# fmfi-compbio/nadavca

Measured on AMD Instinct MI355X. Metric: reads/sec (align_signal, ~4k-sample reads), higher is better.
Workload: dtype f64

## Files before the change

nadavca_amd/csrc/kernels_align3.hip:

```cpp
#include <math.h>

#include <new>
#include <vector>

#include "nvk_internal.h"
#include "xmath.h"
#include "dens.h"
#include "lane3.h"
#include "wave.h"

namespace {

using dens::density;
using dens::density_begin;
using dens::density_end;
using dens::DensHalf;
using dens::ETN;

constexpr int CH = 64;
static_assert(CH == 64, "a refill is one sample per lane");
constexpr int PF = 8;
constexpr int RU = 16;
constexpr int FT = 16;
static_assert(FT % PF == 0 && 32 % FT == 0, "forward trip");
// ... 805 lines not shown
    case 3: return !pair && set_sweeps<MEL, 3, false, TW>(k);
    case 4: return pair ? set_sweeps<MEL, 4, true, TW>(k) : set_sweeps<MEL, 4, false, TW>(k);
    case 5: return pair ? set_sweeps<MEL, 5, true, TW>(k) : set_sweeps<MEL, 5, false, TW>(k);
    default: return false;
  }
}

bool select_sweeps(int mel, bool pair, int W, int rsh, Align3Kernel k[2]) {
  switch (mel) {
    case 0: return sweeps_of<0>(pair, W, rsh, k);
    case 1: return sweeps_of<1>(pair, W, rsh, k);
    case 2: return sweeps_of<2>(pair, W, rsh, k);
    case 3: return sweeps_of<3>(pair, W, rsh, k);
    case 4: return sweeps_of<4>(pair, W, rsh, k);
    default: return false;
  }
}

}

int launch_align3(nvk_ctx *ctx, const BatchArgs &a, int transitions, const ReadMeta *metas, const PlanTotals &tot,
                  const int *order, const int32_t *steps_sorted, int32_t *out_events, int32_t *out_status,
                  int *d_retry) {
  static_assert(WS_OFFS < (int)(sizeof(ctx->ws) / sizeof(ctx->ws[0])), "workspace table too small");
  if (a.n_reads == 0) return NVK_OK;
  const int mel = a.mel;
  if (mel < 0 || mel > 4) {
    nvk_set_error("min_event_length %d outside the compiled range 0..4", mel);
    return NVK_ERR_UNSUPPORTED;
  }
  const int max_c = tot.max_c < 1 ? 1 : tot.max_c;
  int rc = nvk_ws_reserve(ctx, WS_MISC, 256);
  if (rc) return rc;
  int *counter = (int *)ctx->ws[WS_MISC];
  NVK_HIP(hipMemsetAsync(counter, 0, 2 * sizeof(int), ctx->stream));
  NVK_HIP(hipMemsetAsync(d_retry, 0, sizeof(int), ctx->stream));

  constexpr int C_HARD = 24;
  static_assert(ALIGN1_C_CAP + 4 < 8 && C_HARD + 4 < 32, "no kernel for the rescale period these skews need");
  struct Cls { int hi; int W; };
  Cls cls[2];
  int ncls = 0;
  const int64_t n_wide = (int64_t)tot.n_wide;
  const int max_cw = tot.max_cw < 1 ? 1 : tot.max_cw;
  if (a.n_reads - n_wide > 0 || max_c <= ALIGN1_C_CAP)
    cls[ncls++] = Cls{max_c < ALIGN1_C_CAP ? max_c : ALIGN1_C_CAP, 1};
  if (max_c > ALIGN1_C_CAP) cls[ncls++] = Cls{max_cw < C_HARD ? max_cw : C_HARD, ALIGN3_TEAM_W};
  rc = nvk_ws_reserve(ctx, WS_RSTATE, (size_t)a.n_reads * sizeof(int2));
  if (rc) return rc;
  TimerScope ts_align(ctx, NVK_K_ALIGN);
  for (int k = 0; k < ncls; k++) {
    int c = cls[k].hi;
    const int W = cls[k].W, TLk = 64 * W;
    auto lds_need = [&](int cc, int slot_bytes) {
      const int Hc = (cc + mel > 0 ? cc + mel : 1) + (W > 1 ? 1 : 0);
      int SRc = 256;
      while (SRc < 64 * cc + CH) SRc <<= 1;
      return (size_t)ETN * 8 + (size_t)W * SRc * 8 + (size_t)Hc * TLk * slot_bytes + slot_bytes + 16 + 12 * W;
    };
    while (c > 1 && lds_need(c, 20) > 160 * 1024) --c;
    int rsh = transitions ? 4 : 3;
    while ((1 << rsh) <= c + mel) rsh++;
    Align3Kernel kern[2];
    if (!select_sweeps(mel, transitions != 0, W, rsh, kern)) {
      nvk_set_error("no align3 kernel for min_event_length %d, transitions %d, %d waves, rescale period %d", mel,
                    transitions, W, 1 << rsh);
      return NVK_ERR_UNSUPPORTED;
    }
    const int H = (c + mel > 0 ? c + mel : 1) + (W > 1 ? 1 : 0);
    int SR = 256;
    while (SR < 64 * c + CH) SR <<= 1;
    const size_t lds = lds_need(c, 20);
    const size_t lds_rev = lds_need(c, 8);
    if (lds > 160 * 1024) return NVK_ERR_UNSUPPORTED;
    int per_cu = (int)((160 * 1024) / lds);
    if (per_cu > 4 * LB / W) per_cu = 4 * LB / W;
    if (per_cu < 1) per_cu = 1;
    int per_cu_rev = (int)((160 * 1024) / lds_rev);
    if (per_cu_rev > 4 * (W > 1 ? LB_REV_TEAM : LB_REV) / W) per_cu_rev = 4 * (W > 1 ? LB_REV_TEAM : LB_REV) / W;
    if (per_cu_rev < 1) per_cu_rev = 1;
    int32_t mxpad = 1;
    for (int64_t q = 0; q < a.n_reads; q++) mxpad = steps_sorted[q] > mxpad ? steps_sorted[q] : mxpad;
    const int64_t bp_stride = (int64_t)((mxpad + 31) / 32 + 1) * TLk;
    const int64_t cap = nvk_spill_cap(ctx, WS_SPILL);

    Align3Args g;
    g.metas = metas;
    g.fwdl = (const Lane3 *)ctx->ws[WS_LANE_F];
    g.revl = (const Lane3 *)ctx->ws[WS_LANE_R];
    g.offs = (const int32_t *)ctx->ws[WS_OFFS];
    g.signal = a.signal;
    g.bp_stride = bp_stride;
    g.counter = counter;
    g.order = order;
    g.H = H;
    g.SR = SR;
    g.transitions = transitions;
    g.c_cap = c;
    g.flag_above = (k == ncls - 1) ? 1 : 0;
    g.rstate = (int2 *)ctx->ws[WS_RSTATE];
    g.n_retry = d_retry;
    g.ties = (int32_t *)ctx->ws[WS_TIES];
    g.out_events = out_events;
    g.out_status = out_status;
    for (int ph = 0; ph < 2; ph++)
      if ((ph == 0 ? lds_rev : lds) > 64 * 1024)
        NVK_HIP(hipFuncSetAttribute((const void *)kern[ph], hipFuncAttributeMaxDynamicSharedMemorySize,
                                    (int)(ph == 0 ? lds_rev : lds)));
    const int64_t pos_lo = (W > 1) ? 0 : n_wide, pos_hi = (W > 1) ? n_wide : a.n_reads;
    int64_t lo = pos_lo;
    while (lo < pos_hi) {
      int64_t hi = lo, mx = 1;
      while (hi < pos_hi) {
        const int64_t m2 = steps_sorted[hi] > mx ? steps_sorted[hi] : mx;
        if (hi > lo && (m2 + 2 * PF) * 512 * W * (hi - lo + 1) > cap) break;
        mx = m2;
        ++hi;
      }
      int64_t n_chunk = hi - lo;
      int64_t spill_stride = (mx + 2 * PF) * 64;
      while ((rc = nvk_ws_reserve(ctx, WS_SPILL, (size_t)n_chunk * W * spill_stride * 8)) == NVK_ERR_NOMEM &&
             n_chunk > 1) {
        n_chunk = (n_chunk + 1) / 2;
        hi = lo + n_chunk;
        mx = 1;
        for (int64_t q = lo; q < hi; q++) mx = steps_sorted[q] > mx ? steps_sorted[q] : mx;
        spill_stride = (mx + 2 * PF) * 64;
      }
      if (rc) return rc;
      const int64_t L_stride = (mx >> rsh) + 4;
      rc = nvk_ws_reserve(ctx, WS_STAGE, (size_t)n_chunk * L_stride * 4);
      if (rc) return rc;
      int64_t slots_f = ctx->slots_override > 0 ? ctx->slots_override : (int64_t)ctx->num_cus * per_cu;
      int64_t slots_r = ctx->slots_override > 0 ? ctx->slots_override : (int64_t)ctx->num_cus * per_cu_rev;
      if (slots_f > n_chunk) slots_f = n_chunk;
      if (slots_r > n_chunk) slots_r = n_chunk;
      rc = nvk_ws_reserve(ctx, WS_BP, (size_t)slots_f * bp_stride * 4);
      if (rc) return rc;
      g.spill_v = (double *)ctx->ws[WS_SPILL];
      g.spill_L = (int32_t *)ctx->ws[WS_STAGE];
      g.bp = (uint32_t *)ctx->ws[WS_BP];
      g.spill_stride = spill_stride;
      g.L_stride = L_stride;
      g.n_reads = (int)n_chunk;
      g.read_lo = (int)lo;
      NVK_HIP(hipMemsetAsync(counter, 0, sizeof(int), ctx->stream));
      hipLaunchKernelGGL(kern[0], dim3((unsigned)slots_r), dim3(TLk), lds_rev, ctx->stream, g);
      NVK_HIP(hipMemsetAsync(counter, 0, sizeof(int), ctx->stream));
      hipLaunchKernelGGL(kern[1], dim3((unsigned)slots_f), dim3(TLk), lds, ctx->stream, g);
      NVK_HIP(hipGetLastError());
      lo = hi;
    }
  }
  ctx->last_spill_bytes = (int64_t)tot.steps * 64 * 16 + (int64_t)tot.steps / 16 * 8 + (int64_t)tot.steps * 8 * 2;
  return NVK_OK;
}
```

nadavca_amd/csrc/kernels_plan.hip:

```cpp
#include <math.h>

#include "nvk_internal.h"
#include "kmer.h"
#include "lane3.h"
#include "wave.h"

namespace {

__device__ __forceinline__ int read_is_bad(const DeviceModel &dm, const BatchArgs &a, int rd, int tid,
                                           int nthreads) {
  const int64_t s0 = a.sig_off[rd], s1 = a.sig_off[rd + 1], r0 = a.ref_off[rd], r1 = a.ref_off[rd + 1];
  const int64_t a0 = a.anc_off[rd], a1 = a.anc_off[rd + 1];
  const int64_t b0 = a.cb_off[rd], b1 = a.cb_off[rd + 1], c0 = a.ca_off[rd], c1 = a.ca_off[rd + 1];
  const int64_t N64 = s1 - s0, R64 = r1 - r0;
  if (s0 < 0 || r0 < 0 || a0 < 0 || b0 < 0 || c0 < 0 || a1 < a0 || b1 < b0 || c1 < c0 ||
      s1 > a.total_signal || r1 > a.total_ref || a1 > a.total_anchors || b1 - b0 > 0x3fffffff ||
      c1 - c0 > 0x3fffffff)
    return 1;
  if (R64 < 1 || N64 < 1 || N64 > 0x3fffffff || R64 > 0x1fffffff) return 1;
  const int R = (int)R64, A = (int)(a1 - a0), nb = (int)(b1 - b0), na = (int)(c1 - c0);
  const int32_t *anc = a.anchors + 2 * a0;
  const int32_t *ref = a.reference + r0, *cb = a.ctx_before + b0, *ca = a.ctx_after + c0;
  int bad = 0;
  for (int j = tid; j < A && !bad; j += nthreads) {
// ... 30 lines not shown
  }
  __syncthreads();
  int carry = 0;
  for (int base = 0; work && base <= R; base += 64) {
    int j = base + lane;
    int v = 0;
    if (j <= R) {
      unsigned long long w = tbs[j];
      v = (w >> 32) ? (int)(unsigned int)(w & 0xffffffffu) : 0;
    }
    v = max(wave_scan_max(v, lane), carry);
    carry = __shfl(v, 63, 64);
    if (j <= R) tbs[j] = (unsigned long long)(unsigned int)v;
  }
  carry = N;
  for (int base = (R / 64) * 64; work && base >= 0; base -= 64) {
    int j = base + lane;
    int v = N;
    if (j <= R) {
      unsigned long long w = tbe[j];
      v = (w >> 32) ? (int)(unsigned int)(w & 0xffffffffu) - 1 : N;
    } else {
      v = 0x7fffffff;
    }
    v = min(wave_scan_min_rev(v, lane), carry);
    carry = __shfl(v, 0, 64);
    if (j <= R) tbe[j] = (unsigned long long)(unsigned int)v;
  }
  __syncthreads();

}

constexpr int PLAN_T = 256;
__global__ __launch_bounds__(PLAN_T) void plan_kernel(DeviceModel dm, BatchArgs a, int mode,
                                                  double log_p_in, int c_cap, ReadMeta *metas,
                                                  RowParam *rows, unsigned long long *bandtmp,
                                                  PlanTotals *totals, Lane3 *lane_f, Lane3 *lane_r,
                                                  int32_t *lane_offs) {
  const int rd = blockIdx.x;
  const int tid = threadIdx.x, lane = tid & 63;
  __shared__ unsigned long long sh_cells;
  __shared__ int sh_c;
  if (rd >= a.n_reads) return;
  if (tid == 0) {
    sh_cells = 0ull;
    sh_c = 1;
  }
  const int64_t s0 = a.sig_off[rd], r0 = a.ref_off[rd], a0 = a.anc_off[rd];
  const int64_t N64 = a.sig_off[rd + 1] - s0;
  const int64_t R64 = a.ref_off[rd + 1] - r0;
  const int64_t A64 = a.anc_off[rd + 1] - a0;
  const int nb = (int)(a.cb_off[rd + 1] - a.cb_off[rd]);
  const int na = (int)(a.ca_off[rd + 1] - a.ca_off[rd]);
  const int32_t *ref = a.reference + r0;
  const int32_t *cb = a.ctx_before + a.cb_off[rd];
  const int32_t *ca = a.ctx_after + a.ca_off[rd];
  const int32_t *anc = a.anchors + 2 * a0;
  const int N = (int)N64, R = (int)R64, A = (int)A64;
  const int bw = a.bandwidth, mel = a.mel;

  ReadMeta m;
  m.sig_off = s0;
  m.ref_off = r0;
  m.N = N;
  m.R = R;
  m.status = NVK_READ_OK;
  m.pad = 0;
  m.cells = 0;
  m.cw = 0;
  m.rsv = 0;
  int T;
  if (mode == PLAN_ALIGN_TRANS) {
    T = 2 * R;
    m.row_off = 2 * r0;
  } else {
    T = R + 1;
    m.row_off = r0 + rd;
  }
  m.T = T;
  m.c = 1;
  m.t_min = 0;
  m.n_steps = 0;

  int bad = read_is_bad(dm, a, rd, tid, PLAN_T);
  bad = __syncthreads_or(bad);
  if (bad) {
    m.status = NVK_READ_BAD_INPUT;
    if (tid == 0) metas[rd] = m;
    return;
  }

  unsigned long long *tbs = bandtmp + 2 * (r0 + rd);
  unsigned long long *tbe = tbs + (R + 1);
  plan_bands(anc, A, R, N, bw, tbs, tbe, lane, tid < 64);

  RowParam *rp = rows + m.row_off;
  int badband = 0;
  int plateau = 0;
  long long cells = 0;
  for (int r = tid; r < T; r += PLAN_T) {
    RowParam p;
    int bidx = (mode == PLAN_ALIGN_TRANS) ? (r + 1) / 2 : r;
    p.bs = (int)(unsigned int)tbs[bidx];
    p.be = (int)(unsigned int)tbe[bidx];
    if (p.be < p.bs) badband = 1;
    cells += (long long)(p.be - p.bs + 1);
    p.lo = p.bs;
    p.hi = p.be;
    p.mean = 0.0;
    p.ac = 0.0;
    p.mc = 0.0;
    p.mel = 0;
    p.off = 0;
    if (r + 1 < T) {
      if (mode == PLAN_ALIGN_TRANS && (r & 1)) {
        int i = r / 2;
        double m1 = dm.mean[kmer_id(dm, ref, R, cb, nb, ca, na, i)];
        double m2 = dm.mean[kmer_id(dm, ref, R, cb, nb, ca, na, i + 1)];
        p.ac = (m1 == m2) ? -INFINITY : log_p_in;
        p.mel = 0;
        plateau |= (m1 == m2) ? 1 : 0;
      } else {
        int i = (mode == PLAN_ALIGN_TRANS) ? r / 2 : r;
        int64_t id = kmer_id(dm, ref, R, cb, nb, ca, na, i);
        p.mean = dm.mean[id];
        p.ac = dm.ac[id];
        p.mc = dm.mc[id];
        p.mel = mel;
      }
    }
    rp[r] = p;
  }
  badband = __syncthreads_or(badband);
  if (mode != PLAN_ALIGN_TRANS)
    for (int r = tid; r + 2 < T; r += PLAN_T) plateau |= (rp[r].mean == rp[r + 1].mean) ? 1 : 0;
  plateau = __syncthreads_or(plateau);
  cells = wave_sum(cells);
  if (lane == 0) atomicAdd(&sh_cells, (unsigned long long)cells);
  __syncthreads();

  int cneed = 1;
  for (int r = tid; r < T; r += PLAN_T) {
    int lo = rp[r].bs, hi = rp[r].be;
    if (r > 0) {
      int pm = rp[r - 1].mel;
      lo = min(lo, rp[r - 1].bs + pm) - max(pm - 1, 0);
    }
    if (r + 1 < T) {
      int pm = rp[r].mel;
      hi = max(hi, rp[r + 1].be - pm) + max(pm - 1, 0);
    }
    rp[r].lo = lo;
    rp[r].hi = hi;
  }
  __syncthreads();
  const int idle = (mode == PLAN_ALIGN_TRANS) ? 2 : 1;
  for (int r = 64 + tid; r < T; r += PLAN_T) {
    int d = rp[r - 64].hi - rp[r].lo + idle;
    if (d >= 0) cneed = max(cneed, d / 64 + 1);
  }
  cneed = max(cneed, max(mel - 1, 1));
  cneed = wave_max(cneed);
  if (lane == 0) atomicMax(&sh_c, cneed);
  __syncthreads();
  const int c = sh_c;
  cells = (long long)sh_cells;
  const bool team = (c > c_cap);
  int cw = 0;
  if (team) {
    constexpr int TL = 64 * ALIGN3_TEAM_W;
    __shared__ int sh_cw;
    if (tid == 0) sh_cw = max(mel - 1, 1);
    __syncthreads();
    int need = 1;
    for (int r = TL + tid; r < T; r += PLAN_T) {
      int d = rp[r - TL].hi - rp[r].lo + idle;
      if (d >= 0) need = max(need, d / TL + 1);
    }
    need = wave_max(need);
    if (lane == 0) atomicMax(&sh_cw, need);
    __syncthreads();
    cw = sh_cw;
  }

  constexpr int VT = 2048;
  __shared__ int sh_k[VT], sh_x[VT], sh_S[VT];
  __shared__ int sh_var;
  const int gmin = max(mel - 1, 1);
  const bool neg_gaps = (mode == PLAN_ALIGN_TRANS) && mel <= 2;
  if (tid == 0) sh_var = 0;
  __syncthreads();
  if (!team && T <= VT && T > 64 && (neg_gaps || c > gmin)) {
    for (int r = tid; r < T; r += PLAN_T) {
      int g = 0;
      if (r > 0) {
        g = gmin;
        if (neg_gaps) g = max(1 - rp[r - 1].mel, max(rp[r - 1].lo - rp[r].lo, rp[r - 1].hi - rp[r].hi));
        g = min(g, c);
      }
      sh_S[r] = g;
      sh_x[r] = 0;
    }
    __syncthreads();
    if (tid < 64) {
      int carry = 0;
      for (int b0 = 0; b0 < T; b0 += 64) {
        const int r = b0 + lane;
        const int v = wave_scan_add(r < T ? sh_S[r] : 0, lane) + carry;
        if (r < T) sh_S[r] = v;
        carry = __shfl(v, 63, 64);
      }
    }
    __syncthreads();
    for (int r = tid; r < T; r += PLAN_T)
      sh_k[r] = (r >= 64) ? rp[r - 64].hi - rp[r].lo + 1 + idle - (sh_S[r] - sh_S[r - 64]) : 0;
    __syncthreads();
    if (tid < 64) {
      const int NEG = -0x20000000;
      bool changed = true;
      int iter = 0;
      while (changed && iter < 64) {
        changed = false;
        ++iter;
        int carry = 0;
        for (int b0 = 0; b0 < T; b0 += 64) {
          const int r = b0 + lane;
          const int cur = r < T ? sh_x[r] : NEG;
          int v = cur;
          if (r < T && r >= 64) v = max(v, sh_x[r - 64] + sh_k[r]);
          v = max(wave_scan_max(v, lane), carry);
          if (r < T) {
            changed |= (v != cur);
            sh_x[r] = v;
          }
          carry = __shfl(v, 63, 64);
        }
        int carryz = NEG;
        for (int b0 = ((T - 1) / 64) * 64; b0 >= 0; b0 -= 64) {
          const int r = b0 + lane;
          const int cur = r < T ? sh_x[r] : 0;
          const int U = r < T ? c * r - sh_S[r] : 0;
          int z = r < T ? cur - U : NEG;
          z = max(-wave_scan_min_rev(-z, lane), carryz);
          if (r < T) {
            const int nx = z + U;
            changed |= (nx != cur);
            sh_x[r] = nx;
          }
          carryz = __shfl(z, 0, 64);
        }
        changed = __any(changed);
      }
      if (lane == 0) sh_var = changed ? 0 : 1;
    }
    __syncthreads();
  }
  const bool var_ok = (sh_var != 0);
  const int x0 = var_ok ? sh_x[0] : 0;
  const int cu = team ? cw : c;
  for (int r = tid; r < T; r += PLAN_T) rp[r].off = var_ok ? sh_x[r] - x0 + sh_S[r] : cu * r;
  const int off_top = var_ok ? sh_x[T - 1] - x0 + sh_S[T - 1] : cu * (T - 1);
  if (lane_f && !badband) {
    __syncthreads();
    lane3_rows(rp, T, N, cw, lane_f + m.row_off, lane_r + m.row_off, lane_offs + m.row_off, tid, PLAN_T);
  }

  if (tid == 0) {
    int t_min = rp[0].lo;
    int t_max = rp[T - 1].hi + c * (T - 1);
    m.c = c;
    m.cw = cw;
    m.t_min = t_min;
    m.n_steps = t_max - t_min + 1;
    m.pad = rp[T - 1].hi + off_top - t_min + 1;
    m.pad = (m.pad + 31) & ~31;
    m.cells = cells;
    m.rsv = plateau ? 1 : 0;
    if (badband) m.status = NVK_READ_BAD_BAND;
    metas[rd] = m;
    if (!badband) {
      atomicMax(&totals->max_steps, m.n_steps);
      atomicMax(&totals->max_c, c);
      atomicMax(&totals->max_cw, cw);
      if (c > c_cap) atomicAdd(&totals->n_wide, 1);
      atomicMax(&totals->max_T, T);
      atomicAdd(&totals->cells, (unsigned long long)cells);
      atomicAdd(&totals->steps, (unsigned long long)m.pad);
    }
  }
}


__global__ __launch_bounds__(64) void plan_ell_kernel(DeviceModel dm, BatchArgs a, int wobbling,
                                                      EllPlan pl, unsigned long long *bandtmp,
                                                      PlanTotals *totals) {
  const int rd = blockIdx.x;
  const int lane = threadIdx.x;
  if (rd >= a.n_reads) return;
  const int64_t s0 = a.sig_off[rd], r0 = a.ref_off[rd], a0 = a.anc_off[rd];
  const int64_t N64 = a.sig_off[rd + 1] - s0;
  const int64_t R64 = a.ref_off[rd + 1] - r0;
  const int A = (int)(a.anc_off[rd + 1] - a0);
  const int nb = (int)(a.cb_off[rd + 1] - a.cb_off[rd]);
  const int na = (int)(a.ca_off[rd + 1] - a.ca_off[rd]);
  const int32_t *ref = a.reference + r0;
  const int32_t *cb = a.ctx_before + a.cb_off[rd];
  const int32_t *ca = a.ctx_after + a.ca_off[rd];
  const int32_t *anc = a.anchors + 2 * a0;
  const int N = (int)N64, R = (int)R64;

  ReadMeta m;
  m.sig_off = s0;
  m.ref_off = r0;
  m.row_off = r0;
  m.N = N;
  m.R = R;
  m.T = R;
  m.c = 1;
  m.t_min = 0;
  m.n_steps = 0;
  m.status = NVK_READ_OK;
// ... 99 lines not shown
  int64_t g = (int64_t)blockIdx.x * blockDim.x + threadIdx.x;
  if (g >= total_ref) return;
  const int64_t rd = owner_of(ref_off, n_reads, g);
  int R = (int)(ref_off[rd + 1] - ref_off[rd]);
  int nb = (int)(cb_off[rd + 1] - cb_off[rd]);
  int na = (int)(ca_off[rd + 1] - ca_off[rd]);
  int pos = (int)(g - ref_off[rd]);
  const int32_t *ref = reference + ref_off[rd], *cb = cbs + cb_off[rd], *ca = cas + ca_off[rd];
  const int64_t id = kmer_id_checked(dm, ref, R, cb, nb, ca, na, pos);
  out[g] = id >= 0 ? dm.mean[id] : (double)NAN;
}


constexpr int ORD_B = 64;
constexpr int ORD_N = 2 * ORD_B;
__device__ __forceinline__ int order_bucket(const ReadMeta &m, int max_steps) {
  if (m.status != NVK_READ_OK) return ORD_N - 1;
  long long b = (long long)m.n_steps * ORD_B / ((long long)max_steps + 1);
  const int sb = ORD_B - 1 - (int)(b < 0 ? 0 : (b > ORD_B - 1 ? ORD_B - 1 : b));
  return (m.cw != 0 ? 0 : ORD_B) + sb;
}
__global__ void order_count_kernel(const ReadMeta *metas, int n, const PlanTotals *tot, int *cnt) {
  int rd = blockIdx.x * blockDim.x + threadIdx.x;
  if (rd < n) atomicAdd(&cnt[order_bucket(metas[rd], tot->max_steps)], 1);
}
__global__ void order_scan_kernel(int *cnt) {
  int lane = threadIdx.x;
  const int v0 = cnt[2 * lane], v1 = cnt[2 * lane + 1], s = wave_scan_add(v0 + v1, lane);
  cnt[2 * lane] = s - v0 - v1;
  cnt[2 * lane + 1] = s - v1;
  cnt[ORD_N + 2 * lane] = 0;
  cnt[ORD_N + 2 * lane + 1] = 0;
}
__global__ void order_fill_kernel(const ReadMeta *metas, int n, const PlanTotals *tot, int *cnt, int *order) {
  int rd = blockIdx.x * blockDim.x + threadIdx.x;
  if (rd < n) {
    int b = order_bucket(metas[rd], tot->max_steps);
    order[cnt[b] + atomicAdd(&cnt[ORD_N + b], 1)] = rd;
  }
}

__global__ void gather_steps_kernel(const ReadMeta *metas, const int *order, int n, int32_t *out) {
  const int p = blockIdx.x * blockDim.x + threadIdx.x;
  if (p < n) {
    const ReadMeta m = metas[order[p]];
    out[p] = (m.status == NVK_READ_OK) ? m.pad : 0;
  }
}

__global__ void count_flags_kernel(const int32_t *flags, int64_t n, int32_t *out) {
  int64_t g = (int64_t)blockIdx.x * blockDim.x + threadIdx.x;
  const int f = (g < n) ? flags[g] : 0;
  int v = ((f & 7) != 0) ? 1 : 0, v0 = f & 1, v1 = (f >> 1) & 1, v2 = (f >> 2) & 1;
  v = wave_sum(v), v0 = wave_sum(v0), v1 = wave_sum(v1), v2 = wave_sum(v2);
  if ((threadIdx.x & 63) == 0 && v) {
    atomicAdd(out, v);
    if (v0) atomicAdd(out + 1, v0);
    if (v1) atomicAdd(out + 2, v1);
    if (v2) atomicAdd(out + 3, v2);
  }
}

}

int launch_count_flags(nvk_ctx *ctx, const int32_t *flags, int64_t n, int32_t *out_count) {
  NVK_HIP(hipMemsetAsync(out_count, 0, 4 * sizeof(int32_t), ctx->stream));
  if (n <= 0) return NVK_OK;
  hipLaunchKernelGGL(count_flags_kernel, dim3((unsigned)((n + 255) / 256)), dim3(256), 0, ctx->stream, flags, n,
                     out_count);
  NVK_HIP(hipGetLastError());
  return NVK_OK;
}

int launch_order(nvk_ctx *ctx, const ReadMeta *metas, int64_t n_reads, const PlanTotals *tot_dev, int **order,
                 int32_t *steps_out) {
  *order = nullptr;
  if (n_reads <= 0) return NVK_OK;
  int rc = nvk_ws_reserve(ctx, WS_ORDER, (size_t)n_reads * sizeof(int) + 2 * ORD_N * sizeof(int));
  if (rc) return rc;
  int *ord = (int *)ctx->ws[WS_ORDER];
  int *cnt = ord + n_reads;
  NVK_HIP(hipMemsetAsync(cnt, 0, 2 * ORD_N * sizeof(int), ctx->stream));
  const unsigned blocks = (unsigned)((n_reads + 255) / 256);
  TimerScope ts(ctx, NVK_K_PLAN);
  hipLaunchKernelGGL(order_count_kernel, dim3(blocks), dim3(256), 0, ctx->stream, metas, (int)n_reads, tot_dev, cnt);
  hipLaunchKernelGGL(order_scan_kernel, dim3(1), dim3(64), 0, ctx->stream, cnt);
  hipLaunchKernelGGL(order_fill_kernel, dim3(blocks), dim3(256), 0, ctx->stream, metas, (int)n_reads, tot_dev, cnt, ord);
  if (steps_out)
    hipLaunchKernelGGL(gather_steps_kernel, dim3(blocks), dim3(256), 0, ctx->stream, metas, ord, (int)n_reads, steps_out);
  NVK_HIP(hipGetLastError());
  *order = ord;
  return NVK_OK;
}

int launch_plan(nvk_ctx *ctx, const DeviceModel &dm, const BatchArgs &a, int mode,
                ReadMeta *metas, RowParam *rows, unsigned long long *bandtmp, PlanTotals *totals,
                void *lane_f, void *lane_r, int32_t *lane_offs) {
  NVK_HIP(hipMemsetAsync(totals, 0, sizeof(PlanTotals), ctx->stream));
  if (a.n_reads == 0) return NVK_OK;
  {
    TimerScope ts(ctx, NVK_K_PLAN);
    const double log_p_in = log(0.01);
    hipLaunchKernelGGL(plan_kernel, dim3((unsigned)a.n_reads), dim3(PLAN_T), 0, ctx->stream, dm, a, mode,
                       log_p_in, ALIGN1_C_CAP, metas, rows, bandtmp, totals, (Lane3 *)lane_f, (Lane3 *)lane_r,
                       lane_offs);
  }
  NVK_HIP(hipGetLastError());
  return NVK_OK;
}

int launch_plan_ell(nvk_ctx *ctx, const DeviceModel &dm, const BatchArgs &a, int wobbling,
                    const EllPlan &pl, unsigned long long *bandtmp, PlanTotals *totals) {
  NVK_HIP(hipMemsetAsync(totals, 0, sizeof(PlanTotals), ctx->stream));
  if (a.n_reads == 0) return NVK_OK;
  {
    TimerScope ts(ctx, NVK_K_PLAN);
    hipLaunchKernelGGL(plan_ell_kernel, dim3((unsigned)a.n_reads), dim3(64), 0, ctx->stream, dm, a,
                       wobbling, pl, bandtmp, totals);
  }
  NVK_HIP(hipGetLastError());
  return NVK_OK;
}

int launch_expected(nvk_ctx *ctx, const DeviceModel &dm, int64_t n_reads, int64_t total_ref,
                    const int32_t *reference, const int64_t *ref_off, const int32_t *cb,
                    const int64_t *cb_off, const int32_t *ca, const int64_t *ca_off, double *out) {
  if (total_ref == 0) return NVK_OK;
  {
    TimerScope ts(ctx, NVK_K_EXPECTED);
    unsigned blocks = (unsigned)((total_ref + 255) / 256);
    hipLaunchKernelGGL(expected_kernel, dim3(blocks), dim3(256), 0, ctx->stream, dm, n_reads,
                       total_ref, reference, ref_off, cb, cb_off, ca, ca_off, out);
  }
  NVK_HIP(hipGetLastError());
  return NVK_OK;
}
```

nadavca_amd/csrc/lane3.h:

```cpp
#pragma once
#include "nvk_internal.h"
#include "dens.h"

struct __attribute__((aligned(16))) Lane3 {
  double mean, ac, mc;
  int32_t bs;
  int32_t end;
  int32_t lo;
  int32_t pA, pW;
  int32_t mg;
};
__device__ __forceinline__ int lane3_pack(int mel, int age, int adv) { return mel | (age << 4) | (adv * 4096); }
static_assert(sizeof(Lane3) == 48, "Lane3 layout");

__device__ __forceinline__ void set_density_consts(Lane3 &l, const RowParam &o) {
  l.mean = o.mean;
  dens::scale_consts(o.ac, o.mc, l.ac, l.mc);
  if (l.mc == 0.0) l.mean = dens::constant_density(l.ac);
}


__device__ __forceinline__ void lane3_rows(const RowParam *rw, int T, int N, int cw, Lane3 *fwdl, Lane3 *revl,
                                           int32_t *offs, int tid, int nthreads) {
  const int top = T - 1;
  const int ST = cw ? 64 * ALIGN3_TEAM_W : 64;
  for (int r = tid; r < T; r += nthreads) {
    const RowParam o = rw[r];
    Lane3 f, b;
    f.bs = o.bs; f.end = o.be; f.lo = o.lo;
    const int adv_f = (r >= ST) ? o.off - rw[r - ST].off : 0;
    const int adv_b = (r + ST <= top) ? rw[r + ST].off - o.off : 0;
    if (r > 0) {
      const RowParam p = rw[r - 1];
      set_density_consts(f, p);
      f.lo = max(o.lo, p.mel);
      {
        const int a = max(f.lo, p.bs + p.mel), z = min(o.be, p.be + p.mel);
        f.pA = (z >= a) ? a : 0x40000000; f.pW = (z >= a) ? z - a : 0;
      }
      f.mg = lane3_pack(p.mel, o.off - p.off + p.mel, adv_f);
    } else {
      f.mean = 1.0; f.ac = 0.0; f.mc = 0.0; f.mg = lane3_pack(0, 1, 0); f.pA = 0x40000000; f.pW = 0;
    }
    set_density_consts(b, o);
    b.bs = o.bs; b.lo = 0;
    if (r < top) {
      const RowParam q = rw[r + 1];
      b.end = min(o.hi, N - o.mel);
      {
        const int a = max(o.bs, q.bs - o.mel), z = min(b.end, q.be - o.mel);
        b.pA = (z >= a) ? a : 0x40000000; b.pW = (z >= a) ? z - a : 0;
      }
      b.mg = lane3_pack(o.mel, q.off - o.off + o.mel, adv_b);
    } else {
      b.pA = 0x40000000; b.pW = 0;
      b.end = o.hi;
      b.mg = lane3_pack(o.mel, 1 + o.mel, adv_b);
    }
    fwdl[r] = f;
    revl[r] = b;
    offs[r] = o.off;
  }
}
```

nadavca_amd/csrc/wave.h:

```cpp
#pragma once
#include <hip/hip_runtime.h>

#define WAVE_SYNC()                                        \
  do {                                                     \
    __builtin_amdgcn_fence(__ATOMIC_ACQ_REL, "wavefront"); \
    __builtin_amdgcn_wave_barrier();                       \
  } while (0)

__device__ __forceinline__ double dpp_shr1(double v) {
  int lo = __double2loint(v), hi = __double2hiint(v);
  lo = __builtin_amdgcn_mov_dpp(lo, 0x111, 0xf, 0xf, true);
  hi = __builtin_amdgcn_mov_dpp(hi, 0x111, 0xf, 0xf, true);
  return __hiloint2double(hi, lo);
}

__device__ __forceinline__ int dpp_ror1(int v) { return __builtin_amdgcn_mov_dpp(v, 0x13C, 0xf, 0xf, false); }
__device__ __forceinline__ double dpp_ror1(double v) {
  int lo = __double2loint(v), hi = __double2hiint(v);
  lo = __builtin_amdgcn_mov_dpp(lo, 0x13C, 0xf, 0xf, false);
  hi = __builtin_amdgcn_mov_dpp(hi, 0x13C, 0xf, 0xf, false);
  return __hiloint2double(hi, lo);
}

__device__ __forceinline__ int wave_max(int v) {
  for (int d = 32; d >= 1; d >>= 1) v = max(v, __shfl_xor(v, d, 64));
  return v;
}
template <class T>
__device__ __forceinline__ T wave_sum(T v) {
  for (int d = 32; d >= 1; d >>= 1) v += __shfl_xor(v, d, 64);
  return v;
}

__device__ __forceinline__ int wave_scan_add(int v, int lane) {
  for (int d = 1; d < 64; d <<= 1) {
    int o = __shfl_up(v, d, 64);
    if (lane >= d) v += o;
  }
  return v;
}
__device__ __forceinline__ int wave_scan_max(int v, int lane) {
  for (int d = 1; d < 64; d <<= 1) {
    int o = __shfl_up(v, d, 64);
    if (lane >= d) v = max(v, o);
  }
  return v;
}
__device__ __forceinline__ int wave_scan_min_rev(int v, int lane) {
  for (int d = 1; d < 64; d <<= 1) {
    int o = __shfl_down(v, d, 64);
    if (lane + d < 64) v = min(v, o);
  }
  return v;
}
```

Baseline: 648,800.

## Keep per-read planning in LDS, split out totals, trim memsets and scans

Adds an LDS-resident planning path for reads with short references: band scans, kmer ids and offset fixpoint stay in shared memory, and row params and lane records are written in one pass without a global bandtmp round-trip. The totals reduction moves into its own kernel, steps gathering is folded into order_fill, and wave scans use DPP row operations instead of shuffles. The align launcher rotates through a ring of counters so one memset covers many launches instead of one before each. The risks are higher LDS use per plan block, which can lower occupancy, and a second code path that has to match the global one exactly.

```diff
diff --git a/nadavca_amd/csrc/kernels_align3.hip b/nadavca_amd/csrc/kernels_align3.hip
--- a/nadavca_amd/csrc/kernels_align3.hip
+++ b/nadavca_amd/csrc/kernels_align3.hip
@@ -861,8 +861,10 @@
   const int max_c = tot.max_c < 1 ? 1 : tot.max_c;
   int rc = nvk_ws_reserve(ctx, WS_MISC, 256);
   if (rc) return rc;
+  constexpr int N_COUNTERS = 16;
+  static_assert(N_COUNTERS % 2 == 0, "a chunk's reverse / forward pair of counters must not straddle a re-zero");
   int *counter = (int *)ctx->ws[WS_MISC];
-  NVK_HIP(hipMemsetAsync(counter, 0, 2 * sizeof(int), ctx->stream));
+  int launches = 0;
   NVK_HIP(hipMemsetAsync(d_retry, 0, sizeof(int), ctx->stream));
 
   constexpr int C_HARD = 24;
@@ -920,7 +922,6 @@
     g.offs = (const int32_t *)ctx->ws[WS_OFFS];
     g.signal = a.signal;
     g.bp_stride = bp_stride;
-    g.counter = counter;
     g.order = order;
     g.H = H;
     g.SR = SR;
@@ -973,10 +974,12 @@
       g.L_stride = L_stride;
       g.n_reads = (int)n_chunk;
       g.read_lo = (int)lo;
-      NVK_HIP(hipMemsetAsync(counter, 0, sizeof(int), ctx->stream));
+      if (launches % N_COUNTERS == 0) NVK_HIP(hipMemsetAsync(counter, 0, N_COUNTERS * sizeof(int), ctx->stream));
+      g.counter = counter + launches % N_COUNTERS;
       hipLaunchKernelGGL(kern[0], dim3((unsigned)slots_r), dim3(TLk), lds_rev, ctx->stream, g);
-      NVK_HIP(hipMemsetAsync(counter, 0, sizeof(int), ctx->stream));
+      g.counter = counter + (launches + 1) % N_COUNTERS;
       hipLaunchKernelGGL(kern[1], dim3((unsigned)slots_f), dim3(TLk), lds, ctx->stream, g);
+      launches += 2;
       NVK_HIP(hipGetLastError());
       lo = hi;
     }
diff --git a/nadavca_amd/csrc/kernels_plan.hip b/nadavca_amd/csrc/kernels_plan.hip
--- a/nadavca_amd/csrc/kernels_plan.hip
+++ b/nadavca_amd/csrc/kernels_plan.hip
@@ -86,64 +86,339 @@
 }
 
 constexpr int PLAN_T = 256;
-__global__ __launch_bounds__(PLAN_T) void plan_kernel(DeviceModel dm, BatchArgs a, int mode,
-                                                  double log_p_in, int c_cap, ReadMeta *metas,
-                                                  RowParam *rows, unsigned long long *bandtmp,
-                                                  PlanTotals *totals, Lane3 *lane_f, Lane3 *lane_r,
-                                                  int32_t *lane_offs) {
-  const int rd = blockIdx.x;
+constexpr int PLAN_VT = 2048;
+constexpr int PLAN_BCAP = 1024;
+
+struct PlanShared {
+  unsigned long long pool[3 * PLAN_VT / 2];
+  unsigned int ids[PLAN_BCAP];
+  unsigned long long cells;
+  int c, cw, var;
+};
+static_assert(2 * PLAN_BCAP * 8 <= 2 * PLAN_VT * 4 && 2 * PLAN_BCAP <= PLAN_VT, "LDS layout of plan_rows_lds");
+
+struct PlanRead {
+  const int32_t *ref, *cb, *ca, *anc;
+  int64_t r0;
+  int N, R, A, T, nb, na, bw, mel;
+};
+
+__device__ __forceinline__ void plan_bands_lds(const int32_t *anc, int A, int R, int N, int bw,
+                                               unsigned long long *tbs, unsigned long long *tbe, int *bs, int *be,
+                                               int tid) {
+  const int lane = tid & 63, wv = tid >> 6;
+  for (int j = tid; j <= R; j += PLAN_T) {
+    tbs[j] = 0ull;
+    tbe[j] = 0ull;
+  }
+  __syncthreads();
+  for (int j = tid; j < A; j += PLAN_T) {
+    int s = anc[2 * j], ri = anc[2 * j + 1];
+    long long lo = (long long)s - bw;
+    long long hi = (long long)s + bw;
+    unsigned int vbs = (unsigned int)(lo > 0 ? lo : 0);
+    unsigned int vbe = (unsigned int)((hi < N ? (hi < -1 ? -1 : hi) : N) + 1);
+    unsigned long long tag = ((unsigned long long)(j + 1)) << 32;
+    atomicMax(&tbs[ri], tag | vbs);
+    atomicMax(&tbe[ri], tag | vbe);
+  }
+  __syncthreads();
+  if (wv == 0) {
+    int carry = 0;
+    for (int base = 0; base <= R; base += 64) {
+      int j = base + lane;
+      int v = 0;
+      if (j <= R) {
+        unsigned long long w = tbs[j];
+        v = (w >> 32) ? (int)(unsigned int)(w & 0xffffffffu) : 0;
+      }
+      v = max(wave_scan_max_dpp(v), carry);
+      carry = __builtin_amdgcn_readlane(v, 63);
+      if (j <= R) bs[j] = v;
+    }
+  } else if (wv == 1) {
+    int carry = N;
+    for (int base = (R / 64) * 64; base >= 0; base -= 64) {
+      int j = base + 63 - lane;
+      int v = N;
+      if (j <= R) {
+        unsigned long long w = tbe[j];
+        v = (w >> 32) ? (int)(unsigned int)(w & 0xffffffffu) - 1 : N;
+      } else {
+        v = 0x7fffffff;
+      }
+      v = min(wave_scan_min_dpp(v), carry);
+      carry = __builtin_amdgcn_readlane(v, 63);
+      if (j <= R) be[j] = v;
+    }
+  }
+  __syncthreads();
+}
+
+__device__ __forceinline__ void plan_rows_lds(const DeviceModel &dm, const PlanRead &q, int mode, double log_p_in,
+                                              int c_cap, int rd, ReadMeta m, ReadMeta *metas, RowParam *rows,
+                                              Lane3 *lane_f, Lane3 *lane_r, int32_t *lane_offs, PlanShared &sh) {
+  const int tid = threadIdx.x, lane = tid & 63, wv = tid >> 6;
+  const int32_t *ref = q.ref, *cb = q.cb, *ca = q.ca;
+  const int N = q.N, R = q.R, T = q.T, nb = q.nb, na = q.na, mel = q.mel;
+  const bool trans = (mode == PLAN_ALIGN_TRANS);
+  constexpr int VT = PLAN_VT;
+  int *sh_x = (int *)sh.pool, *sh_S = sh_x + VT;
+  int *sh_bs = sh_S + VT, *sh_be = sh_bs + PLAN_BCAP;
+  plan_bands_lds(q.anc, q.A, R, N, q.bw, sh.pool, sh.pool + PLAN_BCAP, sh_bs, sh_be, tid);
+
+  auto rmel = [=](int r) { return (r + 1 < T && !(trans && (r & 1))) ? mel : 0; };
+  auto BS = [=](int r) { return sh_bs[trans ? (r + 1) >> 1 : r]; };
+  auto BE = [=](int r) { return sh_be[trans ? (r + 1) >> 1 : r]; };
+  auto LO = [=](int r) {
+    int lo = BS(r);
+    if (r > 0) {
+      const int pm = rmel(r - 1);
+      lo = min(lo, BS(r - 1) + pm) - max(pm - 1, 0);
+    }
+    return lo;
+  };
+  auto HI = [=](int r) {
+    int hi = BE(r);
+    if (r + 1 < T) {
+      const int pm = rmel(r);
+      hi = max(hi, BE(r + 1) - pm) + max(pm - 1, 0);
+    }
+    return hi;
+  };
+
+  const int idle = trans ? 2 : 1;
+  int badband = 0;
+  long long cells = 0;
+  int cneed = 1;
+  for (int r = tid; r < T; r += PLAN_T) {
+    const int b0 = BS(r), b1 = BE(r);
+    if (b1 < b0) badband = 1;
+    cells += (long long)(b1 - b0 + 1);
+    if (r >= 64) {
+      int d = HI(r - 64) - LO(r) + idle;
+      if (d >= 0) cneed = max(cneed, d / 64 + 1);
+    }
+  }
+  cneed = max(cneed, max(mel - 1, 1));
+  badband = __syncthreads_or(badband);
+  cells = wave_sum(cells);
+  cneed = wave_max(cneed);
+  if (lane == 0) {
+    atomicAdd(&sh.cells, (unsigned long long)cells);
+    atomicMax(&sh.c, cneed);
+  }
+  __syncthreads();
+  const int c = sh.c;
+  cells = (long long)sh.cells;
+  const bool team = (c > c_cap);
+  int cw = 0;
+  if (team) {
+    constexpr int TL = 64 * ALIGN3_TEAM_W;
+    if (tid == 0) sh.cw = max(mel - 1, 1);
+    __syncthreads();
+    int need = 1;
+    for (int r = TL + tid; r < T; r += PLAN_T) {
+      int d = HI(r - TL) - LO(r) + idle;
+      if (d >= 0) need = max(need, d / TL + 1);
+    }
+    need = wave_max(need);
+    if (lane == 0) atomicMax(&sh.cw, need);
+    __syncthreads();
+    cw = sh.cw;
+  }
+
+  const int gmin = max(mel - 1, 1);
+  const bool neg_gaps = trans && mel <= 2;
+  const bool fixp = !team && T <= VT && T > 64 && (neg_gaps || c > gmin);
+  if (tid == 0) sh.var = 0;
+  if (fixp) {
+    for (int r = tid; r < T; r += PLAN_T) {
+      int g = 0;
+      if (r > 0) {
+        g = gmin;
+        if (neg_gaps) g = max(1 - rmel(r - 1), max(LO(r - 1) - LO(r), HI(r - 1) - HI(r)));
+        g = min(g, c);
+      }
+      sh_S[r] = g;
+      sh_x[r] = 0;
+    }
+  }
+  __syncthreads();
+  const int t0 = fixp ? 64 : 0;
+  if (tid >= t0) {
+    for (int i = tid - t0; i < R; i += PLAN_T - t0) sh.ids[i] = (unsigned int)kmer_id(dm, ref, R, cb, nb, ca, na, i);
+  }
+  {
+    if (fixp && tid < 64) {
+      int carry = 0;
+      for (int b0 = 0; b0 < T; b0 += 64) {
+        const int r = b0 + lane;
+        const int v = wave_scan_add_dpp(r < T ? sh_S[r] : 0) + carry;
+        if (r < T) sh_S[r] = v;
+        carry = __builtin_amdgcn_readlane(v, 63);
+      }
+      const int NEG = -0x20000000;
+      bool changed = true;
+      int iter = 0;
+      while (changed && iter < 64) {
+        changed = false;
+        ++iter;
+        int carry = 0;
+        int xup = 0, Sup = 0;
+        int cur_n = lane < T ? sh_x[lane] : NEG, Sr_n = lane < T ? sh_S[lane] : 0, d_n = 0;
+        for (int b0 = 0; b0 < T; b0 += 64) {
+          const int r = b0 + lane;
+          const int cur = cur_n, Sr = Sr_n, d = d_n;
+          if (r + 64 < T) {
+            cur_n = sh_x[r + 64];
+            Sr_n = sh_S[r + 64];
+            d_n = HI(r) - LO(r + 64) + 1 + idle;
+          } else {
+            cur_n = NEG;
+            Sr_n = 0;
+          }
+          int v = cur;
+          if (r < T && r >= 64) {
+            const int k = d - (Sr - Sup);
+            v = max(v, xup + k);
+          }
+          v = max(wave_scan_max_dpp(v), carry);
+          if (r < T) {
+            changed |= (v != cur);
+            sh_x[r] = v;
+          }
+          carry = __builtin_amdgcn_readlane(v, 63);
+          xup = v;
+          Sup = Sr;
+        }
+        WAVE_SYNC();
+        int carryz = NEG;
+        const int rz = ((T - 1) / 64) * 64 + 63 - lane;
+        int curz_n = rz < T ? sh_x[rz] : 0, Sz_n = rz < T ? sh_S[rz] : 0;
+        for (int b0 = ((T - 1) / 64) * 64; b0 >= 0; b0 -= 64) {
+          const int r = b0 + 63 - lane;
+          const int cur = curz_n;
+          const int U = r < T ? c * r - Sz_n : 0;
+          if (b0 >= 64) {
+            curz_n = sh_x[r - 64];
+            Sz_n = sh_S[r - 64];
+          }
+          int z = r < T ? cur - U : NEG;
+          z = max(wave_scan_max_dpp(z), carryz);
+          if (r < T) {
+            const int nx = z + U;
+            changed |= (nx != cur);
+            sh_x[r] = nx;
+          }
+          carryz = __builtin_amdgcn_readlane(z, 63);
+        }
+        WAVE_SYNC();
+        changed = __any(changed);
+      }
+      if (lane == 0) sh.var = changed ? 0 : 1;
+    }
+    __syncthreads();
+  }
+  const bool var_ok = (sh.var != 0);
+  const int x0 = var_ok ? sh_x[0] : 0;
+  const int cu = team ? cw : c;
+  auto OFF = [=](int r) { return var_ok ? sh_x[r] - x0 + sh_S[r] : cu * r; };
+
+  RowParam *rp = rows + m.row_off;
+  const bool records = lane_f && !badband;
+  const int top = T - 1;
+  const int ST = cw ? 64 * ALIGN3_TEAM_W : 64;
+  int plateau = 0;
+  for (int base = 0; base < T; base += 63 * (PLAN_T / 64)) {
+    const int r = base + 63 * wv + lane - 1;
+    const bool have = (r >= 0 && r < T);
+    RowParam o;
+    o.mean = 0.0;
+    o.ac = 0.0;
+    o.mc = 0.0;
+    o.mel = 0;
+    o.bs = o.be = o.lo = o.hi = o.off = 0;
+    if (have && r + 1 < T) {
+      if (trans && (r & 1)) {
+        int i = r / 2;
+        double m1 = dm.mean[sh.ids[i]];
+        double m2 = dm.mean[sh.ids[i + 1]];
+        o.ac = (m1 == m2) ? -INFINITY : log_p_in;
+        plateau |= (m1 == m2) ? 1 : 0;
+      } else {
+        int i = trans ? r / 2 : r;
+        const unsigned int id = sh.ids[i];
+        o.mean = dm.mean[id];
+        o.ac = dm.ac[id];
+        o.mc = dm.mc[id];
+        o.mel = mel;
+      }
+    }
+    RowParam p, nx;
+    p.mean = __shfl_up(o.mean, 1, 64);
+    p.ac = __shfl_up(o.ac, 1, 64);
+    p.mc = __shfl_up(o.mc, 1, 64);
+    p.bs = p.be = p.lo = p.hi = p.mel = p.off = 0;
+    nx.mean = nx.ac = nx.mc = 0.0;
+    nx.bs = nx.be = nx.lo = nx.hi = nx.mel = nx.off = 0;
+    if (have && lane > 0) {
+      o.bs = BS(r);
+      o.be = BE(r);
+      o.lo = LO(r);
+      o.hi = HI(r);
+      o.off = OFF(r);
+      if (!trans && r > 0 && r + 1 < T) plateau |= (p.mean == o.mean) ? 1 : 0;
+      rp[r] = o;
+      if (records) {
+        if (r > 0) {
+          p.bs = BS(r - 1);
+          p.be = BE(r - 1);
+          p.mel = rmel(r - 1);
+          p.off = OFF(r - 1);
+        }
+        if (r < top) {
+          nx.bs = BS(r + 1);
+          nx.be = BE(r + 1);
+          nx.off = OFF(r + 1);
+        }
+        const int adv_f = (r >= ST) ? o.off - OFF(r - ST) : 0;
+        const int adv_b = (r + ST <= top) ? OFF(r + ST) - o.off : 0;
+        Lane3 f, b;
+        lane3_row(o, p, r > 0, nx, r < top, N, adv_f, adv_b, f, b);
+        (lane_f + m.row_off)[r] = f;
+        (lane_r + m.row_off)[r] = b;
+        (lane_offs + m.row_off)[r] = o.off;
+      }
+    }
+  }
+  plateau = __syncthreads_or(plateau);
+
+  if (tid == 0) {
+    const int hi_top = HI(T - 1);
+    int t_min = LO(0);
+    int t_max = hi_top + c * (T - 1);
+    m.c = c;
+    m.cw = cw;
+    m.t_min = t_min;
+    m.n_steps = t_max - t_min + 1;
+    m.pad = hi_top + OFF(T - 1) - t_min + 1;
+    m.pad = (m.pad + 31) & ~31;
+    m.cells = cells;
+    m.rsv = plateau ? 1 : 0;
+    if (badband) m.status = NVK_READ_BAD_BAND;
+    metas[rd] = m;
+  }
+}
+
+__device__ __forceinline__ void plan_rows_global(const DeviceModel &dm, const PlanRead &q, int mode, double log_p_in,
+                                                 int c_cap, int rd, ReadMeta m, ReadMeta *metas, RowParam *rows,
+                                                 unsigned long long *bandtmp, Lane3 *lane_f, Lane3 *lane_r,
+                                                 int32_t *lane_offs, PlanShared &sh) {
   const int tid = threadIdx.x, lane = tid & 63;
-  __shared__ unsigned long long sh_cells;
-  __shared__ int sh_c;
-  if (rd >= a.n_reads) return;
-  if (tid == 0) {
-    sh_cells = 0ull;
-    sh_c = 1;
-  }
-  const int64_t s0 = a.sig_off[rd], r0 = a.ref_off[rd], a0 = a.anc_off[rd];
-  const int64_t N64 = a.sig_off[rd + 1] - s0;
-  const int64_t R64 = a.ref_off[rd + 1] - r0;
-  const int64_t A64 = a.anc_off[rd + 1] - a0;
-  const int nb = (int)(a.cb_off[rd + 1] - a.cb_off[rd]);
-  const int na = (int)(a.ca_off[rd + 1] - a.ca_off[rd]);
-  const int32_t *ref = a.reference + r0;
-  const int32_t *cb = a.ctx_before + a.cb_off[rd];
-  const int32_t *ca = a.ctx_after + a.ca_off[rd];
-  const int32_t *anc = a.anchors + 2 * a0;
-  const int N = (int)N64, R = (int)R64, A = (int)A64;
-  const int bw = a.bandwidth, mel = a.mel;
-
-  ReadMeta m;
-  m.sig_off = s0;
-  m.ref_off = r0;
-  m.N = N;
-  m.R = R;
-  m.status = NVK_READ_OK;
-  m.pad = 0;
-  m.cells = 0;
-  m.cw = 0;
-  m.rsv = 0;
-  int T;
-  if (mode == PLAN_ALIGN_TRANS) {
-    T = 2 * R;
-    m.row_off = 2 * r0;
-  } else {
-    T = R + 1;
-    m.row_off = r0 + rd;
-  }
-  m.T = T;
-  m.c = 1;
-  m.t_min = 0;
-  m.n_steps = 0;
-
-  int bad = read_is_bad(dm, a, rd, tid, PLAN_T);
-  bad = __syncthreads_or(bad);
-  if (bad) {
-    m.status = NVK_READ_BAD_INPUT;
-    if (tid == 0) metas[rd] = m;
-    return;
-  }
-
+  const int32_t *ref = q.ref, *cb = q.cb, *ca = q.ca, *anc = q.anc;
+  const int64_t r0 = q.r0;
+  const int N = q.N, R = q.R, A = q.A, T = q.T, nb = q.nb, na = q.na, bw = q.bw, mel = q.mel;
   unsigned long long *tbs = bandtmp + 2 * (r0 + rd);
   unsigned long long *tbe = tbs + (R + 1);
   plan_bands(anc, A, R, N, bw, tbs, tbe, lane, tid < 64);
@@ -190,7 +465,7 @@
     for (int r = tid; r + 2 < T; r += PLAN_T) plateau |= (rp[r].mean == rp[r + 1].mean) ? 1 : 0;
   plateau = __syncthreads_or(plateau);
   cells = wave_sum(cells);
-  if (lane == 0) atomicAdd(&sh_cells, (unsigned long long)cells);
+  if (lane == 0) atomicAdd(&sh.cells, (unsigned long long)cells);
   __syncthreads();
 
   int cneed = 1;
@@ -215,16 +490,15 @@
   }
   cneed = max(cneed, max(mel - 1, 1));
   cneed = wave_max(cneed);
-  if (lane == 0) atomicMax(&sh_c, cneed);
-  __syncthreads();
-  const int c = sh_c;
-  cells = (long long)sh_cells;
+  if (lane == 0) atomicMax(&sh.c, cneed);
+  __syncthreads();
+  const int c = sh.c;
+  cells = (long long)sh.cells;
   const bool team = (c > c_cap);
   int cw = 0;
   if (team) {
     constexpr int TL = 64 * ALIGN3_TEAM_W;
-    __shared__ int sh_cw;
-    if (tid == 0) sh_cw = max(mel - 1, 1);
+    if (tid == 0) sh.cw = max(mel - 1, 1);
     __syncthreads();
     int need = 1;
     for (int r = TL + tid; r < T; r += PLAN_T) {
@@ -232,17 +506,16 @@
       if (d >= 0) need = max(need, d / TL + 1);
     }
     need = wave_max(need);
-    if (lane == 0) atomicMax(&sh_cw, need);
+    if (lane == 0) atomicMax(&sh.cw, need);
     __syncthreads();
-    cw = sh_cw;
-  }
-
-  constexpr int VT = 2048;
-  __shared__ int sh_k[VT], sh_x[VT], sh_S[VT];
-  __shared__ int sh_var;
+    cw = sh.cw;
+  }
+
+  constexpr int VT = PLAN_VT;
+  int *sh_k = (int *)sh.pool, *sh_x = sh_k + VT, *sh_S = sh_x + VT;
   const int gmin = max(mel - 1, 1);
   const bool neg_gaps = (mode == PLAN_ALIGN_TRANS) && mel <= 2;
-  if (tid == 0) sh_var = 0;
+  if (tid == 0) sh.var = 0;
   __syncthreads();
   if (!team && T <= VT && T > 64 && (neg_gaps || c > gmin)) {
     for (int r = tid; r < T; r += PLAN_T) {
@@ -305,11 +578,11 @@
         }
         changed = __any(changed);
       }
-      if (lane == 0) sh_var = changed ? 0 : 1;
+      if (lane == 0) sh.var = changed ? 0 : 1;
     }
     __syncthreads();
   }
-  const bool var_ok = (sh_var != 0);
+  const bool var_ok = (sh.var != 0);
   const int x0 = var_ok ? sh_x[0] : 0;
   const int cu = team ? cw : c;
   for (int r = tid; r < T; r += PLAN_T) rp[r].off = var_ok ? sh_x[r] - x0 + sh_S[r] : cu * r;
@@ -332,15 +605,108 @@
     m.rsv = plateau ? 1 : 0;
     if (badband) m.status = NVK_READ_BAD_BAND;
     metas[rd] = m;
-    if (!badband) {
-      atomicMax(&totals->max_steps, m.n_steps);
-      atomicMax(&totals->max_c, c);
-      atomicMax(&totals->max_cw, cw);
-      if (c > c_cap) atomicAdd(&totals->n_wide, 1);
-      atomicMax(&totals->max_T, T);
-      atomicAdd(&totals->cells, (unsigned long long)cells);
-      atomicAdd(&totals->steps, (unsigned long long)m.pad);
-    }
+  }
+}
+
+__global__ __launch_bounds__(PLAN_T, 5) void plan_kernel(DeviceModel dm, BatchArgs a, int mode,
+                                                  double log_p_in, int c_cap, ReadMeta *metas,
+                                                  RowParam *rows, unsigned long long *bandtmp,
+                                                  Lane3 *lane_f, Lane3 *lane_r, int32_t *lane_offs) {
+  const int rd = blockIdx.x;
+  const int tid = threadIdx.x;
+  __shared__ PlanShared sh;
+  if (rd >= a.n_reads) return;
+  if (tid == 0) {
+    sh.cells = 0ull;
+    sh.c = 1;
+  }
+  const int64_t s0 = a.sig_off[rd], r0 = a.ref_off[rd], a0 = a.anc_off[rd];
+  const int64_t N64 = a.sig_off[rd + 1] - s0;
+  const int64_t R64 = a.ref_off[rd + 1] - r0;
+  const int64_t A64 = a.anc_off[rd + 1] - a0;
+  PlanRead q;
+  q.nb = (int)(a.cb_off[rd + 1] - a.cb_off[rd]);
+  q.na = (int)(a.ca_off[rd + 1] - a.ca_off[rd]);
+  q.ref = a.reference + r0;
+  q.cb = a.ctx_before + a.cb_off[rd];
+  q.ca = a.ctx_after + a.ca_off[rd];
+  q.anc = a.anchors + 2 * a0;
+  q.r0 = r0;
+  q.N = (int)N64;
+  q.R = (int)R64;
+  q.A = (int)A64;
+  q.bw = a.bandwidth;
+  q.mel = a.mel;
+
+  ReadMeta m;
+  m.sig_off = s0;
+  m.ref_off = r0;
+  m.N = q.N;
+  m.R = q.R;
+  m.status = NVK_READ_OK;
+  m.pad = 0;
+  m.cells = 0;
+  m.cw = 0;
+  m.rsv = 0;
+  if (mode == PLAN_ALIGN_TRANS) {
+    q.T = 2 * q.R;
+    m.row_off = 2 * r0;
+  } else {
+    q.T = q.R + 1;
+    m.row_off = r0 + rd;
+  }
+  m.T = q.T;
+  m.c = 1;
+  m.t_min = 0;
+  m.n_steps = 0;
+
+  int bad = read_is_bad(dm, a, rd, tid, PLAN_T);
+  bad = __syncthreads_or(bad);
+  if (bad) {
+    m.status = NVK_READ_BAD_INPUT;
+    if (tid == 0) metas[rd] = m;
+    return;
+  }
+  if (q.R + 1 <= PLAN_BCAP && dm.n <= 0x100000000ll)
+    plan_rows_lds(dm, q, mode, log_p_in, c_cap, rd, m, metas, rows, lane_f, lane_r, lane_offs, sh);
+  else
+    plan_rows_global(dm, q, mode, log_p_in, c_cap, rd, m, metas, rows, bandtmp, lane_f, lane_r, lane_offs, sh);
+}
+
+__global__ __launch_bounds__(256) void plan_totals_kernel(const ReadMeta *metas, int n, int c_cap, PlanTotals *totals) {
+  const int rd = blockIdx.x * 256 + threadIdx.x, lane = threadIdx.x & 63, wv = threadIdx.x >> 6;
+  int steps = 0, c = 0, cw = 0, T = 0, wide = 0;
+  unsigned long long cells = 0ull, pad = 0ull;
+  if (rd < n) {
+    const ReadMeta m = metas[rd];
+    if (m.status == NVK_READ_OK) {
+      steps = max(m.n_steps, 0), c = max(m.c, 0), cw = max(m.cw, 0), T = max(m.T, 0);
+      wide = (m.c > c_cap) ? 1 : 0;
+      cells = (unsigned long long)m.cells;
+      pad = (unsigned long long)m.pad;
+    }
+  }
+  __shared__ int sh_i[4][5];
+  __shared__ unsigned long long sh_u[4][2];
+  steps = wave_max(steps), c = wave_max(c), cw = wave_max(cw), T = wave_max(T), wide = wave_sum(wide);
+  cells = wave_sum(cells), pad = wave_sum(pad);
+  if (lane == 0) {
+    sh_i[wv][0] = steps, sh_i[wv][1] = c, sh_i[wv][2] = cw, sh_i[wv][3] = T, sh_i[wv][4] = wide;
+    sh_u[wv][0] = cells, sh_u[wv][1] = pad;
+  }
+  __syncthreads();
+  if (threadIdx.x == 0) {
+    for (int w = 1; w < 4; w++) {
+      steps = max(steps, sh_i[w][0]), c = max(c, sh_i[w][1]), cw = max(cw, sh_i[w][2]), T = max(T, sh_i[w][3]);
+      wide += sh_i[w][4], cells += sh_u[w][0], pad += sh_u[w][1];
+    }
+    if (steps) atomicMax(&totals->max_steps, steps);
+    if (c) atomicMax(&totals->max_c, c);
+    if (cw) atomicMax(&totals->max_cw, cw);
+    if (wide) atomicAdd(&totals->n_wide, wide);
+    if (T) atomicMax(&totals->max_T, T);
+    if (cells) atomicAdd(&totals->cells, cells);
+    if (pad) atomicAdd(&totals->steps, pad);
   }
 }
 
@@ -506,19 +872,15 @@
   cnt[ORD_N + 2 * lane] = 0;
   cnt[ORD_N + 2 * lane + 1] = 0;
 }
-__global__ void order_fill_kernel(const ReadMeta *metas, int n, const PlanTotals *tot, int *cnt, int *order) {
+__global__ void order_fill_kernel(const ReadMeta *metas, int n, const PlanTotals *tot, int *cnt, int *order,
+                                  int32_t *steps_out) {
   int rd = blockIdx.x * blockDim.x + threadIdx.x;
   if (rd < n) {
-    int b = order_bucket(metas[rd], tot->max_steps);
-    order[cnt[b] + atomicAdd(&cnt[ORD_N + b], 1)] = rd;
-  }
-}
-
-__global__ void gather_steps_kernel(const ReadMeta *metas, const int *order, int n, int32_t *out) {
-  const int p = blockIdx.x * blockDim.x + threadIdx.x;
-  if (p < n) {
-    const ReadMeta m = metas[order[p]];
-    out[p] = (m.status == NVK_READ_OK) ? m.pad : 0;
+    const ReadMeta m = metas[rd];
+    int b = order_bucket(m, tot->max_steps);
+    const int pos = cnt[b] + atomicAdd(&cnt[ORD_N + b], 1);
+    order[pos] = rd;
+    if (steps_out) steps_out[pos] = (m.status == NVK_READ_OK) ? m.pad : 0;
   }
 }
 
@@ -559,9 +921,8 @@
   TimerScope ts(ctx, NVK_K_PLAN);
   hipLaunchKernelGGL(order_count_kernel, dim3(blocks), dim3(256), 0, ctx->stream, metas, (int)n_reads, tot_dev, cnt);
   hipLaunchKernelGGL(order_scan_kernel, dim3(1), dim3(64), 0, ctx->stream, cnt);
-  hipLaunchKernelGGL(order_fill_kernel, dim3(blocks), dim3(256), 0, ctx->stream, metas, (int)n_reads, tot_dev, cnt, ord);
-  if (steps_out)
-    hipLaunchKernelGGL(gather_steps_kernel, dim3(blocks), dim3(256), 0, ctx->stream, metas, ord, (int)n_reads, steps_out);
+  hipLaunchKernelGGL(order_fill_kernel, dim3(blocks), dim3(256), 0, ctx->stream, metas, (int)n_reads, tot_dev, cnt, ord,
+                     steps_out);
   NVK_HIP(hipGetLastError());
   *order = ord;
   return NVK_OK;
@@ -576,8 +937,9 @@
     TimerScope ts(ctx, NVK_K_PLAN);
     const double log_p_in = log(0.01);
     hipLaunchKernelGGL(plan_kernel, dim3((unsigned)a.n_reads), dim3(PLAN_T), 0, ctx->stream, dm, a, mode,
-                       log_p_in, ALIGN1_C_CAP, metas, rows, bandtmp, totals, (Lane3 *)lane_f, (Lane3 *)lane_r,
-                       lane_offs);
+                       log_p_in, ALIGN1_C_CAP, metas, rows, bandtmp, (Lane3 *)lane_f, (Lane3 *)lane_r, lane_offs);
+    hipLaunchKernelGGL(plan_totals_kernel, dim3((unsigned)((a.n_reads + 255) / 256)), dim3(256), 0, ctx->stream,
+                       metas, (int)a.n_reads, ALIGN1_C_CAP, totals);
   }
   NVK_HIP(hipGetLastError());
   return NVK_OK;
diff --git a/nadavca_amd/csrc/lane3.h b/nadavca_amd/csrc/lane3.h
--- a/nadavca_amd/csrc/lane3.h
+++ b/nadavca_amd/csrc/lane3.h
@@ -20,6 +20,36 @@
 }
 
 
+__device__ __forceinline__ void lane3_row(const RowParam &o, const RowParam &p, bool has_p, const RowParam &q,
+                                          bool has_q, int N, int adv_f, int adv_b, Lane3 &f, Lane3 &b) {
+  f.bs = o.bs; f.end = o.be; f.lo = o.lo;
+  if (has_p) {
+    set_density_consts(f, p);
+    f.lo = max(o.lo, p.mel);
+    {
+      const int a = max(f.lo, p.bs + p.mel), z = min(o.be, p.be + p.mel);
+      f.pA = (z >= a) ? a : 0x40000000; f.pW = (z >= a) ? z - a : 0;
+    }
+    f.mg = lane3_pack(p.mel, o.off - p.off + p.mel, adv_f);
+  } else {
+    f.mean = 1.0; f.ac = 0.0; f.mc = 0.0; f.mg = lane3_pack(0, 1, 0); f.pA = 0x40000000; f.pW = 0;
+  }
+  set_density_consts(b, o);
+  b.bs = o.bs; b.lo = 0;
+  if (has_q) {
+    b.end = min(o.hi, N - o.mel);
+    {
+      const int a = max(o.bs, q.bs - o.mel), z = min(b.end, q.be - o.mel);
+      b.pA = (z >= a) ? a : 0x40000000; b.pW = (z >= a) ? z - a : 0;
+    }
+    b.mg = lane3_pack(o.mel, q.off - o.off + o.mel, adv_b);
+  } else {
+    b.pA = 0x40000000; b.pW = 0;
+    b.end = o.hi;
+    b.mg = lane3_pack(o.mel, 1 + o.mel, adv_b);
+  }
+}
+
 __device__ __forceinline__ void lane3_rows(const RowParam *rw, int T, int N, int cw, Lane3 *fwdl, Lane3 *revl,
                                            int32_t *offs, int tid, int nthreads) {
   const int top = T - 1;
@@ -27,36 +57,9 @@
   for (int r = tid; r < T; r += nthreads) {
     const RowParam o = rw[r];
     Lane3 f, b;
-    f.bs = o.bs; f.end = o.be; f.lo = o.lo;
     const int adv_f = (r >= ST) ? o.off - rw[r - ST].off : 0;
     const int adv_b = (r + ST <= top) ? rw[r + ST].off - o.off : 0;
-    if (r > 0) {
-      const RowParam p = rw[r - 1];
-      set_density_consts(f, p);
-      f.lo = max(o.lo, p.mel);
-      {
-        const int a = max(f.lo, p.bs + p.mel), z = min(o.be, p.be + p.mel);
-        f.pA = (z >= a) ? a : 0x40000000; f.pW = (z >= a) ? z - a : 0;
-      }
-      f.mg = lane3_pack(p.mel, o.off - p.off + p.mel, adv_f);
-    } else {
-      f.mean = 1.0; f.ac = 0.0; f.mc = 0.0; f.mg = lane3_pack(0, 1, 0); f.pA = 0x40000000; f.pW = 0;
-    }
-    set_density_consts(b, o);
-    b.bs = o.bs; b.lo = 0;
-    if (r < top) {
-      const RowParam q = rw[r + 1];
-      b.end = min(o.hi, N - o.mel);
-      {
-        const int a = max(o.bs, q.bs - o.mel), z = min(b.end, q.be - o.mel);
-        b.pA = (z >= a) ? a : 0x40000000; b.pW = (z >= a) ? z - a : 0;
-      }
-      b.mg = lane3_pack(o.mel, q.off - o.off + o.mel, adv_b);
-    } else {
-      b.pA = 0x40000000; b.pW = 0;
-      b.end = o.hi;
-      b.mg = lane3_pack(o.mel, 1 + o.mel, adv_b);
-    }
+    lane3_row(o, rw[r > 0 ? r - 1 : r], r > 0, rw[r < top ? r + 1 : r], r < top, N, adv_f, adv_b, f, b);
     fwdl[r] = f;
     revl[r] = b;
     offs[r] = o.off;
diff --git a/nadavca_amd/csrc/wave.h b/nadavca_amd/csrc/wave.h
--- a/nadavca_amd/csrc/wave.h
+++ b/nadavca_amd/csrc/wave.h
@@ -53,3 +53,25 @@
   }
   return v;
 }
+
+#define WAVE_SCAN_DPP_STEP(ctrl, rows) v = op(v, __builtin_amdgcn_update_dpp(ident, v, ctrl, rows, 0xf, false))
+template <class Op>
+__device__ __forceinline__ int wave_scan_dpp(int v, const int ident, Op op) {
+  WAVE_SCAN_DPP_STEP(0x111, 0xf);
+  WAVE_SCAN_DPP_STEP(0x112, 0xf);
+  WAVE_SCAN_DPP_STEP(0x114, 0xf);
+  WAVE_SCAN_DPP_STEP(0x118, 0xf);
+  WAVE_SCAN_DPP_STEP(0x142, 0xa);
+  WAVE_SCAN_DPP_STEP(0x143, 0xc);
+  return v;
+}
+#undef WAVE_SCAN_DPP_STEP
+__device__ __forceinline__ int wave_scan_add_dpp(int v) {
+  return wave_scan_dpp(v, 0, [](int a, int b) { return a + b; });
+}
+__device__ __forceinline__ int wave_scan_max_dpp(int v) {
+  return wave_scan_dpp(v, (int)0x80000000, [](int a, int b) { return max(a, b); });
+}
+__device__ __forceinline__ int wave_scan_min_dpp(int v) {
+  return wave_scan_dpp(v, 0x7fffffff, [](int a, int b) { return min(a, b); });
+}
```

After: 671,300, median of 6. 1.03x the previous value.
